# astaka-pe/SeMIGCN

Hardware: AMD Instinct MI355X
Metric: GCN train iters/sec + edges-aggregated/sec, 1M-vert mesh (higher is better)
Workload: dtype bf16 storage / f32 accumulate; 1 GPU; SGCN train iteration (13 ChebConv K=3 + BN + LeakyReLU, fwd+loss+bwd, Adam every 5th) on a closed torus mesh 1000x1000: V=1000000 E=6000000 directed, grid vertex order, bf16 features; V=1000000, E=6000000, vertex_order=grid

## Files before the change

### include/semigcn.h

```cpp
#ifndef SEMIGCN_H
#define SEMIGCN_H

#include <stdint.h>

#ifdef __cplusplus
extern "C" {
#endif

#if defined(__GNUC__)
#define SG_API __attribute__((visibility("default")))
#else
#define SG_API
#endif

#define SG_ABI_VERSION 1

enum sg_status {
  SG_OK = 0,
  SG_ERR_INVALID = -1,
  SG_ERR_HIP = -2,
  SG_ERR_UNSUPPORTED = -3,
  SG_ERR_NO_DEVICE = -4
};

// ... 182 lines not shown
SG_API int64_t sg_bnf_blocks(int64_t F);
SG_API int64_t sg_bnf_scratch_bytes(int64_t F);
SG_API int sg_bnf_filter(const float* pos, const int64_t* faces, const int64_t* f2f, int64_t V, int64_t F, int loop,
                         float sigma_s, const float* start_fn, float* fn, float* n_filtered, float* loss_partial,
                         void* scratch, void* stream);
SG_API int sg_mesh_loss_cad_finalize(const float* partial, int64_t nb, float n_v, float n_f, float w_pos, float k1,
                                     const float* bnf_partial, int64_t nb_bnf, int64_t F, float k2, float* out, void* stream);
SG_API int sg_mesh_loss_cad_bwd_det(const float* pos, const int64_t* faces, const float* target_pos, const float* v_keep,
                                    const float* target_fn, const float* f_keep, const float* fn, const float* n_filtered,
                                    const float* g, int64_t V, int64_t V_ext, int64_t F, const sg_pool* incidence,
                                    float* corner_scratch, float* grad_pos, void* stream);

SG_API int sg_gemm_nt_takes_big_tile(int64_t M, int64_t N, int64_t K, int64_t lda, int64_t ldb, int64_t ldc);
SG_API int64_t sg_gemm_tile_rows(int64_t N);
SG_API int64_t sg_gemm_row_tiles(int64_t M, int64_t N);
SG_API int sg_gemm_nt(const void* A, int64_t lda, const void* B, int64_t ldb, const float* bias, void* C, int64_t ldc,
                      int64_t M, int64_t N, int64_t K, int dtype, float* moments, void* stream);
SG_API int64_t sg_gemm_tn_slabs(int64_t M, int64_t N, int64_t Kp);
SG_API int sg_gemm_tn_takes_big_tile(int64_t M, int64_t N, int64_t Kp, int64_t lda, int64_t ldb);
SG_API int sg_gemm_tn(const void* A, int64_t lda, const void* B, int64_t ldb, int64_t M, int64_t N, int64_t Kp, int dtype,
                      float* workspace, float* out, int64_t ldo, void* stream);
SG_API int sg_gemm_nt_f32_supported(int64_t M, int64_t N, int64_t K, int64_t lda, int64_t ldc);
SG_API int sg_gemm_nt_f32_pays(int64_t M, int64_t N, int64_t K);
SG_API int sg_gemm_nt_f32_variant(int64_t M);
SG_API int64_t sg_gemm_nt_f32_workspace(int64_t N, int64_t K);
SG_API int sg_gemm_nt_f32(const float* A, int64_t lda, const float* W, int64_t w_rs, int64_t w_cs, const float* bias, float* C,
                          int64_t ldc, int64_t M, int64_t N, int64_t K, void* workspace, int64_t workspace_bytes, void* stream);
SG_API int sg_gemm_tn_f32_supported(int64_t M, int64_t N, int64_t Kp, int64_t lda, int64_t ldb);
SG_API int64_t sg_gemm_tn_f32_workspace(int64_t M, int64_t N, int64_t Kp);
SG_API int sg_gemm_tn_f32(const float* A, int64_t lda, const float* B, int64_t ldb, int64_t M, int64_t N, int64_t Kp,
// ... 147 lines not shown
```

### semigcn_amd/capi.py

```python
from __future__ import annotations

import ctypes
import functools
from array import array as _array
import os
from ctypes import POINTER, byref, c_char_p, c_float, c_int, c_int32, c_int64, c_void_p
from typing import Optional

import torch

_LIB_NAME = "libsemigcn_hip.so"
_LIB_PATH = os.path.join(os.path.dirname(os.path.abspath(__file__)), _LIB_NAME)

SG_F32, SG_BF16 = 0, 1
_DTYPES = {torch.float32: SG_F32, torch.bfloat16: SG_BF16}


class SemigcnLibraryError(RuntimeError):
    """libsemigcn_hip.so is absent / unloadable, or a call into it failed."""


class sg_graph_info(ctypes.Structure):
    _fields_ = [("V_dst", c_int64), ("V_src", c_int64), ("nnz", c_int64),
                ("symmetric", c_int32), ("max_degree", c_int32)]
# ... 61 lines not shown
    "sg_tuning_set": (c_int, [c_int, c_int]),
    "sg_mesh_loss_blocks": (c_int64, [c_int64, c_int64]),
    "sg_mesh_loss_fwd": (c_int, [c_void_p] * 6 + [c_int64, c_int64, c_void_p, c_void_p]),
    "sg_mesh_loss_bwd": (c_int, [c_void_p] * 7 + [c_int64, c_int64, c_int64, c_void_p, c_void_p]),
    "sg_mesh_loss_bwd_det": (c_int, [c_void_p] * 7 + [c_int64, c_int64, c_int64, c_void_p, c_void_p, c_void_p, c_void_p]),
    "sg_col_blocks": (c_int64, [c_int64]),
    "sg_col_moments": (c_int, [c_void_p, c_int64, c_int64, c_int64, c_int, c_void_p, c_int64, c_void_p]),
    "sg_bn_merge": (c_int, [c_void_p, c_int64, c_int64, c_int64, c_void_p, c_void_p]),
    "sg_bn_stats_finalize": (c_int, [c_void_p, c_int64, c_int64, c_int64, c_void_p, c_void_p, c_void_p, c_void_p, c_float,
                                     c_float, c_void_p, c_void_p, c_void_p]),
    "sg_bn_stats_finalize_tiles": (c_int, [c_void_p, c_int64, c_int64, c_int64, c_int64, c_void_p, c_void_p, c_void_p,
                                           c_void_p, c_float, c_float, c_void_p, c_void_p, c_void_p]),
    "sg_gemm_nt_takes_big_tile": (c_int, [c_int64, c_int64, c_int64, c_int64, c_int64, c_int64]),
    "sg_gemm_tile_rows": (c_int64, [c_int64]),
    "sg_gemm_row_tiles": (c_int64, [c_int64, c_int64]),
    "sg_gemm_nt": (c_int, [c_void_p, c_int64, c_void_p, c_int64, c_void_p, c_void_p, c_int64, c_int64, c_int64, c_int64,
                           c_int, c_void_p, c_void_p]),
    "sg_gemm_nt_f32_supported": (c_int, [c_int64, c_int64, c_int64, c_int64, c_int64]),
    "sg_gemm_nt_f32_pays": (c_int, [c_int64, c_int64, c_int64]),
    "sg_gemm_nt_f32_variant": (c_int, [c_int64]),
    "sg_gemm_nt_f32_workspace": (c_int64, [c_int64, c_int64]),
    "sg_gemm_nt_f32": (c_int, [c_void_p, c_int64, c_void_p, c_int64, c_int64, c_void_p, c_void_p, c_int64, c_int64, c_int64,
                               c_int64, c_void_p, c_int64, c_void_p]),
    "sg_gemm_tn_f32_supported": (c_int, [c_int64, c_int64, c_int64, c_int64, c_int64]),
    "sg_gemm_tn_f32_workspace": (c_int64, [c_int64, c_int64, c_int64]),
    "sg_gemm_tn_f32": (c_int, [c_void_p, c_int64, c_void_p, c_int64, c_int64, c_int64, c_int64, c_void_p, c_int64, c_void_p,
                               c_int64, c_void_p]),
    "sg_gemm_tn_slabs": (c_int64, [c_int64, c_int64, c_int64]),
    "sg_gemm_tn_takes_big_tile": (c_int, [c_int64, c_int64, c_int64, c_int64, c_int64]),
    "sg_gemm_tn": (c_int, [c_void_p, c_int64, c_void_p, c_int64, c_int64, c_int64, c_int64, c_int, c_void_p, c_void_p, c_int64,
# ... 577 lines not shown
        if t is not None:
            _f32vec(t, C, n)
    with _on_device(partial.device):
        _check(load().sg_bn_stats_finalize_tiles(_ptr(partial), nb, int(rows_per_tile), int(num_rows), C,
                                                 _ptr(_f32vec(gamma, C, "weight")), _ptr(_f32vec(beta, C, "bias")),
                                                 _ptr(running_mean), _ptr(running_var), float(momentum), float(eps),
                                                 _ptr(out), _counter(batches_tracked, partial), _stream(partial)),
               "sg_bn_stats_finalize_tiles")
    return out


def gemm_tile_rows(N: int) -> int:
    return _sizes("sg_gemm_tile_rows", int(N))


def gemm_nt_supported(A: torch.Tensor, B: torch.Tensor, ldc: int) -> bool:
    if A.dtype != torch.bfloat16 or B.dtype != torch.bfloat16 or not A.is_cuda or A.dim() != 2 or B.dim() != 2:
        return False
    if A.shape[1] != B.shape[1] or A.stride(1) != 1 or B.stride(1) != 1 or A.shape[0] == 0:
        return False
    K, N = A.shape[1], B.shape[0]
    return (K % 8 == 0 and N % 8 == 0 and A.stride(0) % 8 == 0 and B.stride(0) % 8 == 0 and ldc % 8 == 0
            and A.data_ptr() % 16 == 0 and B.data_ptr() % 16 == 0)


def gemm_nt_takes_big_tile(M: int, N: int, K: int, lda: int, ldb: int, ldc: int) -> bool:
    return bool(_sizes("sg_gemm_nt_takes_big_tile", int(M), int(N), int(K), int(lda), int(ldb), int(ldc)))


def gemm_nt(A: torch.Tensor, B: torch.Tensor, bias: Optional[torch.Tensor] = None, out: Optional[torch.Tensor] = None,
            moments: bool = False):
    _require_device(A, "A")
    _require_device(B, "B")
    M, K = A.shape
    N = B.shape[0]
    if out is None:
        out = torch.empty((M, N), dtype=torch.bfloat16, device=A.device)
    if out.shape != (M, N) or out.dtype != torch.bfloat16 or B.shape[1] != K:
        raise SemigcnLibraryError(f"gemm_nt shape mismatch: A {tuple(A.shape)} B {tuple(B.shape)} out {tuple(out.shape)}")
    if bias is not None:
        _f32vec(bias, N, "bias")
    mom = None
    if moments:
        mom = torch.empty((_sizes("sg_gemm_row_tiles", M, N), 2, N), dtype=torch.float32, device=A.device)
    with _on_device(A.device):
        _check(load().sg_gemm_nt(_ptr(A), _rows2d(A, "A"), _ptr(B), _rows2d(B, "B"), _ptr(bias), _ptr(out),
                                 _rows2d(out, "out"), M, N, K, SG_BF16, _ptr(mom), _stream(A)), "sg_gemm_nt")
    return (out, mom) if moments else out


THIN_ELEMS = 256


def thin_shape(N: int, K: int) -> bool:
    return bool(_sizes("sg_thin_supported", int(N), int(K)))


def thin_supported(A: torch.Tensor, N: int, K: int) -> bool:
    return (A.is_cuda and A.dim() == 2 and A.stride(1) == 1 and A.dtype in (torch.float32, torch.bfloat16)
# ... 1120 lines not shown
```

### semigcn_amd/csrc/api.hip

```cpp
#include <stdarg.h>

#include <new>

#include <mutex>

#include "sg_common.h"

namespace sg {

static thread_local std::string t_error;

void set_error(const char* fmt, ...) {
  char buf[1024];
  va_list ap;
  va_start(ap, fmt);
  vsnprintf(buf, sizeof(buf), fmt, ap);
  va_end(ap);
  t_error = buf;
}

namespace {

struct ScopedFree {
  void* p = nullptr;
// ... 777 lines not shown
  return launch_bn_stats_finalize_tiles(partial, n_tiles, rows_per_tile, V, C, gamma, beta, running_mean, running_var,
                                        momentum, eps, out, batches_tracked, (hipStream_t)stream);
}

SG_API int sg_gemm_nt_takes_big_tile(int64_t M, int64_t N, int64_t K, int64_t lda, int64_t ldb, int64_t ldc) {
  return gemm_nt_takes_big_tile(M, N, K, lda, ldb, ldc) ? 1 : 0;
}

SG_API int64_t sg_gemm_tile_rows(int64_t N) { return gemm_tile_rows(N); }

SG_API int64_t sg_gemm_row_tiles(int64_t M, int64_t N) {
  const int64_t r = gemm_tile_rows(N);
  return M <= 0 ? 0 : (M + r - 1) / r;
}

SG_API int sg_gemm_nt(const void* A, int64_t lda, const void* B, int64_t ldb, const float* bias, void* C, int64_t ldc,
                      int64_t M, int64_t N, int64_t K, int dtype, float* moments, void* stream) {
  SG_REQUIRE(M >= 0 && N >= 0 && K >= 0, "sg_gemm_nt: negative size");
  if (M == 0 || N == 0) return SG_OK;
  SG_REQUIRE(A && B && C && K > 0, "sg_gemm_nt: null operand or K = 0");
  SG_REQUIRE(lda >= K && ldb >= K && ldc >= N, "sg_gemm_nt: row stride shorter than the row");
  return launch_gemm_nt(A, lda, B, ldb, bias, C, ldc, M, N, K, dtype, moments, (hipStream_t)stream);
}

SG_API int64_t sg_gemm_tn_slabs(int64_t M, int64_t N, int64_t Kp) { return gemm_tn_slabs(M, N, Kp); }

SG_API int sg_gemm_tn_takes_big_tile(int64_t M, int64_t N, int64_t Kp, int64_t lda, int64_t ldb) {
  return gemm_tn_takes_big_tile(M, N, Kp, lda, ldb) ? 1 : 0;
}

// ... 269 lines not shown
```

### semigcn_amd/csrc/block.hip

```cpp
#include <math.h>

#include "sg_common.h"

namespace sg {
namespace {

bool g_block_planes = true;

inline int64_t esize(int dtype) { return dtype == SG_F32 ? 4 : 2; }
inline int64_t align_up(int64_t v) { return (v + 255) & ~(int64_t)255; }

struct Carver {
  char* base;
  int64_t cap, at = 0;
  bool overflow = false;
  Carver(void* b, int64_t c) : base((char*)b), cap(c) {}
  void* take(int64_t bytes) {
    const int64_t off = at;
    at += align_up(bytes > 0 ? bytes : 1);
    if (!base) return nullptr;
    if (at > cap) {
      overflow = true;
      return nullptr;
    }
// ... 47 lines not shown
  if (c >= C) return;
  const float mean = rm[c];
  const float invstd = rsqrtf(__fadd_rn(rv[c], eps));
  const float scale = __fmul_rn(gamma[c], invstd);
  out[c] = mean;
  out[C + c] = invstd;
  out[2 * C + c] = scale;
  out[3 * C + c] = __fsub_rn(beta[c], __fmul_rn(mean, scale));
}

int copy_rows(const void* src, int64_t lds, void* dst, int64_t ldd, int64_t rows, int64_t cols, int dtype, hipStream_t s) {
  const int64_t e = esize(dtype);
  SG_HIP_TRY(hipMemcpy2DAsync(dst, (size_t)(ldd * e), src, (size_t)(lds * e), (size_t)(cols * e), (size_t)rows,
                              hipMemcpyDeviceToDevice, s));
  return SG_OK;
}

struct Shape {
  int64_t V, Vo, Ci, Co, KCi, KCo, e;
  int K;
  bool thin, blas_fwd, blas_dx, blas_dw;
  bool planes_ok;
  Planes pl;
  int64_t nb;
  int64_t mom_floats;
  int64_t tn_floats;
};

int shape_of(const sg_block& b, Shape* s) {
  SG_REQUIRE(b.graph != nullptr, "sg_block: null graph");
// ... 46 lines not shown
    bool ok = b.dtype == SG_BF16 && b.K > 1 && (1 << lg) == C && C >= 8 && C <= 64 && g_block_planes;
    if (ok && b.order == 0)
      ok = dense_planes_ok_nt(b.dtype, s->V, s->Co, s->KCi) && dense_planes_ok_nt(b.dtype, s->V, s->KCi, s->Co) &&
           dense_planes_ok_tn(b.dtype, s->V, s->Co, s->KCi);
    else if (ok)
      ok = dense_planes_ok_nt(b.dtype, s->V, s->KCo, s->Ci) && dense_planes_ok_nt(b.dtype, s->V, s->Ci, s->KCo) &&
           dense_planes_ok_tn(b.dtype, s->V, s->KCo, s->Ci);
    s->planes_ok = ok;
    s->pl = Planes{};
    if (ok) {
      s->pl.log2 = lg;
      s->pl.stride = s->V * C;
    }
  }
  s->nb = col_blocks(s->Vo);
  const int64_t R = gemm_tile_rows(s->Co);
  const int64_t tiles = (s->V + R - 1) / R;
  s->mom_floats = (tiles > s->nb ? tiles : s->nb) * 2 * s->Co;
  return SG_OK;
}

struct FwdWs {
  float* moments;
  void* Z;
  void* Hc;
  void* blas;
};
void carve_fwd(const sg_block& b, const Shape& s, Carver& c, FwdWs* w) {
  w->moments = (float*)c.take(s.mom_floats * 4);
  w->Z = b.order == 1 ? c.take(s.V * s.KCo * s.e) : nullptr;
  w->Hc = b.pool_mode ? c.take(s.V * s.Co * s.e) : nullptr;
  w->blas = s.blas_fwd ? c.take((int64_t)kBlasWorkspace) : nullptr;
// ... 112 lines not shown
    auto z = [&](int k) { return pz.on() ? col(w.Z, k * pz.stride, s.e) : col(w.Z, k * s.Co, s.e); };
    for (int k = b.K - 2; k >= 1; --k) {
      rc = spmm(b, false, z(k + 1), ldz, z(k), ldz, k + 2 <= b.K - 1 ? z(k + 2) : nullptr, ldz, z(k), ldz, s.Co, 2.f, 1.f, -1.f,
                stream);
      if (rc != SG_OK) return rc;
    }
    rc = spmm(b, false, z(1), ldz, z(0), ldz, b.K >= 3 ? z(2) : nullptr, ldz, Hc, s.Co, s.Co, 1.f, 1.f, -1.f, stream);
    if (rc != SG_OK) return rc;
  }
  if (b.pool_mode == 1) rc = sg_pool_mean(b.pool, Hc, s.Co, b.H, s.Co, s.Co, b.dtype, (void*)stream);
  else if (b.pool_mode == 2) rc = sg_unpool(b.pool, Hc, s.Co, b.H, s.Co, s.Co, b.dtype, (void*)stream);
  if (rc != SG_OK) return rc;

  if (b.training) {
    if (tile_moments) {
      const int64_t R = gemm_tile_rows(s.Co);
      rc = launch_bn_stats_finalize_tiles(w.moments, (s.V + R - 1) / R, R, s.Vo, s.Co, b.gamma, b.beta, b.running_mean,
                                          b.running_var, b.momentum, b.eps, b.stats, b.batches_tracked, stream);
    } else {
      rc = launch_col_reduce(0, b.H, s.Co, nullptr, 0, nullptr, nullptr, nullptr, nullptr, 0.f, w.moments, s.nb, s.Vo, s.Co,
                             b.dtype, stream);
      if (rc != SG_OK) return rc;
      rc = launch_bn_stats_finalize(w.moments, s.nb, s.Vo, s.Co, b.gamma, b.beta, b.running_mean, b.running_var, b.momentum,
                                    b.eps, b.stats, b.batches_tracked, stream);
    }
    if (rc != SG_OK) return rc;
  } else {
    bn_eval_coeffs<<<(int)((s.Co + 127) / 128), 128, 0, stream>>>(b.running_mean, b.running_var, b.gamma, b.beta, b.eps,
                                                                 (int)s.Co, b.stats);
    SG_HIP_TRY(hipGetLastError());
  }
// ... 174 lines not shown
  return SG_OK;
}

struct PartWs {
  float* moments;
  void* Z;
  float* part;
  float* co;
  float* colsum;
  void* dH;
  float* tn;
  void* blas;
};
void carve_part(const sg_block& b, Carver& c, PartWs* w) {
  const int64_t e = esize(b.dtype), KCi = b.K * b.Cin, KCo = b.K * b.Cout;
  const int64_t nb = col_blocks(b.V), R = gemm_tile_rows(b.Cout), tiles = (b.V + R - 1) / R;
  w->moments = (float*)c.take((tiles > nb ? tiles : nb) * 2 * b.Cout * 4);
  w->Z = b.order == 1 ? c.take(b.V_ext * KCo * e) : nullptr;
  w->part = (float*)c.take(nb * 2 * b.Cout * 4);
  w->co = (float*)c.take(5 * b.Cout * 4);
  w->colsum = (float*)c.take(col_apply_blocks(b.V, b.Cout, b.dtype) * b.Cout * 4);
  w->dH = b.order == 0 ? c.take(b.V * b.Cout * e) : nullptr;
  const int64_t tn = b.order == 0 ? dense_tn_workspace(b.dtype, b.V, b.Cout, KCi) : dense_tn_workspace(b.dtype, b.V, KCo, b.Cin);
  w->tn = (float*)c.take(tn * 4);
  w->blas = c.take((int64_t)kBlasWorkspace);
}

int pack_to(const sg_block& b, const void* src, int64_t ld, int64_t width, const float* blob, int64_t blob_floats, hipStream_t stream) {
  if (b.n_send == 0) return SG_OK;
  SG_REQUIRE(b.send && b.send_index, "sg_block_run: no send buffer / index");
  const int64_t e = esize(b.dtype);
// ... 37 lines not shown
      if (rc != SG_OK) return rc;
    } else {
      SG_REQUIRE(b.X && b.ldx >= Ci, "sg_block_run (conv): order 1 needs the [V_ext, Cin] input X");
      if (b.bias) SG_REQUIRE(b.bias_k != nullptr, "sg_block_run (conv): order 1 with a bias needs bias_k");
      rc = dense_nt(b.X, b.ldx, b.wpack, nullptr, Ci, b.bias ? b.bias_k : nullptr, w.Z, KCo, Ve, KCo, Ci, b.dtype, nullptr, nullptr,
                    w.blas, kBlasWorkspace, stream, Planes{}, Planes{}, split_image(b, false, KCo, Ci), b.V);
      if (rc != SG_OK) return rc;
      char* z0 = (char*)w.Z;
      char* z1 = col(w.Z, Co, e);
      char* z2 = col(w.Z, 2 * Co, e);
      if ((rc = agg(b.graph_wide, z2, KCo, z1, KCo, nullptr, 0, z1, KCo, Co, 2.f, 1.f, 0.f)) != SG_OK) return rc;
      if ((rc = agg(b.graph, z1, KCo, z0, KCo, z2, KCo, b.H, b.ldh, Co, 1.f, 1.f, -1.f)) != SG_OK) return rc;
    }
    if (b.training) {
      if (tile_moments) {
        const int64_t R = gemm_tile_rows(Co);
        rc = launch_bn_merge_tiles(w.moments, (V + R - 1) / R, R, V, Co, b.local, b.local + 2 * Co, stream);
      } else {
        const int64_t nb = col_blocks(V);
        rc = launch_col_reduce(0, b.H, b.ldh, nullptr, 0, nullptr, nullptr, nullptr, nullptr, 0.f, w.moments, nb, V, Co, b.dtype, stream);
        if (rc != SG_OK) return rc;
        rc = launch_bn_merge_tiles(w.moments, nb, (V + nb - 1) / nb, V, Co, b.local, b.local + 2 * Co, stream);
      }
      if (rc != SG_OK) return rc;
    }
    if (b.n_send > 0 && (rc = pack_to(b, b.H, b.ldh, Co, b.training ? b.local : nullptr, 2 * Co + 1, stream)) != SG_OK) return rc;
  }

  if (b.phase & SG_PHASE_BN) {
    SG_REQUIRE(b.stats && b.gamma && b.beta && b.Y && b.ldy >= Co && b.V_out >= V && b.V_out <= Ve, "sg_block_run (bn): bad argument");
    if (b.training) {
// ... 210 lines not shown
```

### semigcn_amd/csrc/dense.hip

```cpp
#include <dlfcn.h>

#include <map>
#include <mutex>
#include <tuple>

#include <hipblaslt/hipblaslt.h>

#include "sg_common.h"

namespace sg {
namespace {

struct LtApi {
  decltype(&hipblasLtCreate) Create = nullptr;
  decltype(&hipblasLtMatmulDescCreate) DescCreate = nullptr;
  decltype(&hipblasLtMatmulDescSetAttribute) DescSet = nullptr;
  decltype(&hipblasLtMatrixLayoutCreate) LayoutCreate = nullptr;
  decltype(&hipblasLtMatrixLayoutSetAttribute) LayoutSet = nullptr;
  decltype(&hipblasLtMatmulPreferenceCreate) PrefCreate = nullptr;
  decltype(&hipblasLtMatmulPreferenceSetAttribute) PrefSet = nullptr;
  decltype(&hipblasLtMatmulPreferenceDestroy) PrefDestroy = nullptr;
  decltype(&hipblasLtMatmulAlgoGetHeuristic) Heuristic = nullptr;
  decltype(&hipblasLtMatmul) Matmul = nullptr;
  decltype(&hipblasLtGetVersion) GetVersion = nullptr;
// ... 224 lines not shown
  if (moments_done) *moments_done = false;
  if (M == 0 || N == 0) return SG_OK;
  if (pa.on() || pc.on()) {
    SG_REQUIRE(dense_planes_ok_nt(dtype, M, N, K) && a16(A) && a16(Bp) && a16(C),
               "dense_nt: an operand kept as planes for a product the 128-row kernel does not serve (M=%lld N=%lld K=%lld)",
               (long long)M, (long long)N, (long long)K);
    if (moments_done) *moments_done = moments != nullptr;
    TraceScope ts(1, dtype, 1, M, N, K, stream);
    return launch_gemm_nt(A, lda, Bp, ldb, bias, C, ldc, M, N, K, dtype, moments, stream, pa, pc);
  }
  if (thin_shape(N, K) && B32) {
    TraceScope ts(1, dtype, 2, M, N, K, stream);
    return launch_thin_nt(A, lda, B32, ldb, bias, C, ldc, M, N, K, dtype, stream);
  }
  if (dense_nt_own(dtype, M, N, K, lda, ldb, ldc) && a16(A) && a16(Bp) && a16(C)) {
    const bool big = gemm_nt_takes_big_tile(M, N, K, lda, ldb, ldc);
    float* mom = (moments && !big) ? moments : nullptr;
    if (moments_done) *moments_done = mom != nullptr;
    TraceScope ts(1, dtype, 1, M, N, K, stream);
    return launch_gemm_nt(A, lda, Bp, ldb, bias, C, ldc, M, N, K, dtype, mom, stream);
  }
  if (dtype == SG_F32 && split_engine_enabled(0) && split_nt_pays(M, N, K) && gemm_nt_f32s_supported(M, N, K, lda, ldc) && a16(A) && a16(C) &&
      (presplit || (blas_ws && (int64_t)blas_ws_bytes >= gemm_nt_f32s_workspace(N, K)))) {
    TraceScope ts(1, dtype, 4, M, N, K, stream);
    return launch_gemm_nt_f32s((const float*)A, lda, (const float*)Bp, ldb, 1, bias, (float*)C, ldc, M, N, K, blas_ws,
                               (int64_t)blas_ws_bytes, stream, presplit, presplit_rows);
  }
  if (dtype == SG_F32 && split_engine_enabled(0) && mid_shape(N, K) && lda % 4 == 0 && ldc % 4 == 0 && a16(A) && a16(C)) {
    TraceScope ts(1, dtype, 2, M, N, K, stream);
    return launch_mid_nt((const float*)A, lda, (const float*)Bp, ldb, 1, bias, (float*)C, ldc, M, N, K, stream);
  }
  TraceScope ts(1, dtype, 3, M, N, K, stream);
  return lt_gemm(0, 1, M, N, K, A, lda, Bp, ldb, bias, C, ldc, dtype, dtype, 1, 0, 0, 0, blas_ws, blas_ws_bytes, stream);
}

// ... 100 lines not shown
```

### semigcn_amd/csrc/gemm_mfma.hip

```cpp
#include "sg_common.h"

namespace sg {
namespace {

typedef __attribute__((ext_vector_type(8))) __bf16 bf16x8;
typedef __attribute__((ext_vector_type(4))) float f32x4;
typedef uint32_t u32x4 __attribute__((ext_vector_type(4)));

constexpr int kThreads = 256;
constexpr int kBK = 64;
constexpr int kRowBytes = 128;

struct GemmArgs {
  const uint16_t* A; int64_t lda;
  const uint16_t* B; int64_t ldb;
  const float* bias;
  uint16_t* C; int64_t ldc;
  float* moments;
  int M, N, K;
  int n_col_tiles, n_tiles;
  int a_plog; int64_t a_pstride;
  int c_plog; int64_t c_pstride;
};

// ... 233 lines not shown
constexpr int64_t kBigMinWeightElems = 90000;
constexpr int64_t kBigMinRows = 16384;

bool wide_tile(int64_t N) { return g_gemm_tile == 2 && N > 64; }
bool tile_192(int64_t N) { return g_gemm_tile != 1 && g_gemm_tile != 4 && (N == 192 || (g_gemm_tile == 5 && N == 384)); }

}

int gemm_tile_rows(int64_t N) { return wide_tile(N) ? 64 : 128; }

bool gemm_nt_takes_big_tile(int64_t M, int64_t N, int64_t K, int64_t lda, int64_t ldb, int64_t ldc) {
  if (g_gemm_tile == 1 || g_gemm_tile == 2 || !gemm_nt_256_supported(M, N, K, lda, ldb, ldc)) return false;
  return g_gemm_tile == 3 || (K * N > kBigMinWeightElems && M >= kBigMinRows);
}

int set_gemm_tuning(int value) {
  g_gemm_tile = value;
  return SG_OK;
}

int launch_gemm_nt(const void* A, int64_t lda, const void* B, int64_t ldb, const float* bias, void* C, int64_t ldc,
                   int64_t M, int64_t N, int64_t K, int dtype, float* moments, hipStream_t stream, Planes pa, Planes pc) {
  if (dtype != SG_BF16) {
    set_error("sg_gemm_nt: bf16 operands only (dtype %d); fp32 products stay with the BLAS library", dtype);
    return SG_ERR_UNSUPPORTED;
  }
  if (K % 8 || N % 8 || lda % 8 || ldb % 8 || ldc % 8 || !a16(A) || !a16(B) || !a16(C)) {
    set_error("sg_gemm_nt: needs K, N and the row strides to be multiples of 8 and 16-byte aligned operands "
              "(K=%lld N=%lld lda=%lld ldb=%lld ldc=%lld)", (long long)K, (long long)N, (long long)lda, (long long)ldb,
              (long long)ldc);
    return SG_ERR_UNSUPPORTED;
  }
  SG_REQUIRE(M <= INT32_MAX && N <= INT32_MAX && K <= INT32_MAX, "sg_gemm_nt: size out of range");
  const bool planes = pa.on() || pc.on();
  if (planes) {
    SG_REQUIRE((!pa.on() || (pa.log2 >= 3 && pa.log2 < 31 && pa.stride % 8 == 0)) &&
               (!pc.on() || (pc.log2 >= 3 && pc.log2 < 31 && pc.stride % 8 == 0)),
               "sg_gemm_nt: planes need >= 8 columns each and a plane stride that is a multiple of 8 elements");
    SG_REQUIRE(!wide_tile(N), "sg_gemm_nt: operands kept as planes run on the 128-row tiles only");
  }
  if (!planes && moments == nullptr && gemm_nt_takes_big_tile(M, N, K, lda, ldb, ldc))
    return launch_gemm_nt_256(A, lda, B, ldb, bias, C, ldc, M, N, K, stream);
  GemmArgs g;
  g.a_plog = pa.log2; g.a_pstride = pa.stride;
  g.c_plog = pc.log2; g.c_pstride = pc.stride;
  g.A = (const uint16_t*)A; g.lda = lda;
  g.B = (const uint16_t*)B; g.ldb = ldb;
  g.bias = bias;
  g.C = (uint16_t*)C; g.ldc = ldc;
  g.moments = moments;
  g.M = (int)M; g.N = (int)N; g.K = (int)K;
  g.n_col_tiles = g.n_tiles = 0;
  if (wide_tile(N)) return launch<1, 4, 4, 4>(g, stream);
  if (tile_192(N) && !moments) return launch<2, 2, 4, 6>(g, stream);
  if (N > 64) return launch<2, 2, 4, 4>(g, stream);
  if (N > 32) return launch<4, 1, 2, 4>(g, stream);
  if (N > 16) return launch<4, 1, 2, 2>(g, stream);
// ... 247 lines not shown
```

### semigcn_amd/csrc/gemm_mfma256.hip

```cpp
#include "sg_common.h"

namespace sg {
namespace {

typedef __attribute__((ext_vector_type(8))) __bf16 bf16x8;
typedef __attribute__((ext_vector_type(4))) float f32x4;
typedef uint32_t u32x2 __attribute__((ext_vector_type(2)));
typedef uint32_t u32x4 __attribute__((ext_vector_type(4)));
typedef float f32x2 __attribute__((ext_vector_type(2)));
typedef __attribute__((ext_vector_type(4))) __bf16 bf16x4;
typedef __bf16 bf16x2 __attribute__((ext_vector_type(2)));

constexpr int kThreads256 = 512;
constexpr int kHalf = 16384;
constexpr int kBuf = 4 * kHalf;
constexpr int AH0 = 0, AH1 = 1, BH0 = 2, BH1 = 3;

struct Big {
  const uint16_t* A; int64_t lda;
  const uint16_t* B; int64_t ldb;
  const float* bias;
  uint16_t* C; int64_t ldc;
  int M, N, K;
  int n_col_tiles, n_row_tiles, streams;
#ifdef SG_GEMM256_STAMPS
  unsigned long long* stamps;
#endif
};

#if defined(SG_GEMM256_STAMPS) && !defined(SG_G256_NOSTAMP)
#define SG_STAMP(ph, k)                                                                                         \
  if (blockIdx.x == 8 && (wave == 0 || wave == 4) && lane == 0 && s >= 16 && s < 32)                              \
    ((unsigned long long*)(lds + 2 * kBuf))[(((wave >> 2) * 16 + (s - 16)) * 4 + (ph)) * 6 + (k)] = __builtin_readcyclecounter();
#else
#define SG_STAMP(ph, k)
#endif

// ... 33 lines not shown
[[maybe_unused]] __device__ __forceinline__ bf16x8 sg_fake_frag(const uint8_t* p) {
  bf16x8 v;
  asm volatile("" : "=v"(v) : "v"(p));
  return v;
}

__device__ __forceinline__ void glds16(const void* src, uint8_t* lds_dst) {
#ifdef SG_G256_NOLOAD
  asm volatile("" ::"v"(src), "s"(lds_dst));
  return;
#endif
  __builtin_amdgcn_global_load_lds((const void __attribute__((address_space(1)))*)src,
                                   (void __attribute__((address_space(3)))*)lds_dst, 16, 0, 0);
}

__global__ __launch_bounds__(kThreads256, 1) void gemm_nt_256(const Big g) {
#ifdef SG_GEMM256_STAMPS
  __shared__ __attribute__((aligned(1024))) uint8_t lds[2 * kBuf + 2 * 16 * 4 * 6 * 8];
#else
  __shared__ __attribute__((aligned(1024))) uint8_t lds[2 * kBuf];
#endif

  const int tid = threadIdx.x, lane = tid & 63;
  const int wave = __builtin_amdgcn_readfirstlane(tid >> 6);
  const int wr = wave >> 2, wc = wave & 3;
  const int fr = lane & 15, fq = lane >> 4;

  const int b = blockIdx.x;
  const int slot = b >> 3;
  const int ct = slot % g.n_col_tiles;
// ... 84 lines not shown
  load_a(0, 0);
  load_b(0, 0);
  load_b(1, 0);
  load_a(1, 0);
  advance();
  load_a(0, 1);
  load_b(0, 1);
  SG_WAIT_VM(8);
  SG_BARRIER();
  if (wr == 1) SG_BARRIER2();

  int since = 2;
  int pend_row0 = 0;
  auto store_quadrant = [&](int q) {
    const int i0 = q >= 2 ? 4 : 0, jp = (q == 1 || q == 2) ? 1 : 0;
#pragma unroll
    for (int ii = 0; ii < 4; ++ii) {
      const int i = i0 + ii;
      const int row = pend_row0 + (i >> 2) * 128 + wr * 64 + (i & 3) * 16 + fr;
      uint16_t* const cptr = g.C + (int64_t)row * g.ldc + col0 + wc * 32 + (fq & 1) * 16 + (fq >> 1) * 8 + jp * 128;
      uint32_t lo[2], hi[2];
#pragma unroll
      for (int jj = 0; jj < 2; ++jj) {
        const int j = 2 * jp + jj;
        lo[jj] = __builtin_bit_cast(uint32_t, __builtin_convertvector(f32x2{acc[i][j][0], acc[i][j][1]}, bf16x2));
        hi[jj] = __builtin_bit_cast(uint32_t, __builtin_convertvector(f32x2{acc[i][j][2], acc[i][j][3]}, bf16x2));
        acc[i][j] = bias_v[j];
      }
      const auto ra = __builtin_amdgcn_permlane16_swap(lo[0], lo[1], false, false);
      const auto rb = __builtin_amdgcn_permlane16_swap(hi[0], hi[1], false, false);
      if (row < g.M) SG_STORE16(cptr, (u32x4{ra[0], rb[0], ra[1], rb[1]}));
    }
  };
#define SG_PHASE_WAIT(n0, n1)                 \
  if (since == 0) SG_WAIT_VM(n0);             \
  else SG_WAIT_VM(n1);

  bf16x8 af[4][2], bf0[2][2], bf1[2][2];
  int ct_k = 0, ct_t = 0;
  for (int s = 0; s < total; ++s) {
    const int buf = s & 1;
    const uint8_t* const base = lds + buf * kBuf;
    SG_STAMP(0, 0)
#pragma unroll
    for (int j = 0; j < 2; ++j)
#pragma unroll
      for (int ks = 0; ks < 2; ++ks) bf0[j][ks] = SG_LDS_FRAG(base + BH0 * kHalf + b_rd[ks] + j * 2048);
#pragma unroll
    for (int i = 0; i < 4; ++i)
#pragma unroll
      for (int ks = 0; ks < 2; ++ks) af[i][ks] = SG_LDS_FRAG(base + AH0 * kHalf + a_rd[ks] + i * 2048);
// ... 286 lines not shown
#pragma unroll
      for (int r = 0; r < 4; ++r) {
        const int n = n0 + (i >> 2) * 128 + wr * 64 + (i & 3) * 16 + fg * 4 + r;
        W[(int64_t)n * g.Kp + kk] = acc[i][j][r];
      }
    }
}

}

bool gemm_nt_256_supported(int64_t M, int64_t N, int64_t K, int64_t lda, int64_t ldb, int64_t ldc) {
  return K >= 128 && K % 64 == 0 && N >= 256 && N % 256 == 0 && M >= 256 && lda % 8 == 0 && ldb % 8 == 0 && ldc % 8 == 0 &&
         256 * lda * 2 < (int64_t)1 << 31 && 256 * ldb * 2 < (int64_t)1 << 31;
}

int launch_gemm_nt_256(const void* A, int64_t lda, const void* B, int64_t ldb, const float* bias, void* C, int64_t ldc,
                       int64_t M, int64_t N, int64_t K, hipStream_t stream) {
  SG_REQUIRE(gemm_nt_256_supported(M, N, K, lda, ldb, ldc), "sg_gemm_nt (256-tile kernel): unsupported shape");
  SG_REQUIRE((((uintptr_t)A | (uintptr_t)B) & 15) == 0 && ((uintptr_t)C & 15) == 0, "sg_gemm_nt (256-tile kernel): misaligned operand");
  Big g;
  g.A = (const uint16_t*)A; g.lda = lda;
  g.B = (const uint16_t*)B; g.ldb = ldb;
  g.bias = bias;
  g.C = (uint16_t*)C; g.ldc = ldc;
  g.M = (int)M; g.N = (int)N; g.K = (int)K;
  g.n_col_tiles = (int)(N / 256);
  g.n_row_tiles = (int)((M + 255) / 256);
  int dev = 0, cus = 256;
  SG_HIP_TRY(hipGetDevice(&dev));
  SG_HIP_TRY(hipDeviceGetAttribute(&cus, hipDeviceAttributeMultiprocessorCount, dev));
  int streams = (cus / g.n_col_tiles) / 8 * 8;
  streams = streams < 8 ? 8 : streams;
  const int need = (g.n_row_tiles + 7) / 8 * 8;
  streams = streams > need ? need : streams;
  g.streams = streams;
  gemm_nt_256<<<streams * g.n_col_tiles, kThreads256, 0, stream>>>(g);
  SG_HIP_TRY(hipGetLastError());
  return SG_OK;
}

bool gemm_tn_256_supported(int64_t M, int64_t N, int64_t Kp, int64_t lda, int64_t ldb) {
  return M >= 64 * 64 && N >= 256 && N % 256 == 0 && Kp >= 256 && Kp % 256 == 0 && lda % 8 == 0 && ldb % 8 == 0 &&
         64 * lda * 2 < (int64_t)1 << 31 && 64 * ldb * 2 < (int64_t)1 << 31;
}

int gemm_tn_256_slabs(int64_t M, int64_t N, int64_t Kp) {
  const int n_tiles = (int)((N / 256) * (Kp / 256));
  int slabs = (256 / n_tiles) / 8 * 8;
  slabs = slabs < 8 ? 8 : slabs;
  const int64_t steps = M / 64;
  while (slabs > 8 && steps < slabs) slabs -= 8;
// ... 22 lines not shown
```

### semigcn_amd/csrc/sg_common.h

```cpp
#pragma once
#include <hip/hip_runtime.h>
#include <stdint.h>
#include <stdio.h>
#include <atomic>
#include <string>

#include "semigcn.h"

namespace sg {

void set_error(const char* fmt, ...);

#define SG_HIP_TRY(expr)                                                              \
  do {                                                                                \
    hipError_t e__ = (expr);                                                          \
    if (e__ != hipSuccess) {                                                          \
      sg::set_error("%s failed: %s (%s:%d)", #expr, hipGetErrorString(e__), __FILE__, \
                    __LINE__);                                                        \
      return SG_ERR_HIP;                                                              \
    }                                                                                 \
  } while (0)

#define SG_REQUIRE(cond, ...)      \
  do {                             \
// ... 194 lines not shown
int launch_input_prep_bwd(const void* gX, int64_t ldg, const float* z1, const float* dm, const int64_t* rank, const float* lo,
                          const float* hi, float* dz1, float* partial, float* d_lo, float* d_hi, int64_t V, int dtype,
                          hipStream_t stream);

int launch_input_bounds(const float* z1, int64_t V, float* pv, int64_t* pi, float* bounds, int64_t* arg, hipStream_t stream);
int launch_bounds_route(const float* d_lo, const float* d_hi, const int64_t* arg, float* dz1, hipStream_t stream);
int launch_mesh_loss_finalize(const float* partial, int64_t nb, float n_v, float n_f, float w_pos, float k1, float* out,
                              hipStream_t stream);

int gemm_tile_rows(int64_t N);
int set_gemm_tuning(int value);
int launch_gemm_nt(const void* A, int64_t lda, const void* B, int64_t ldb, const float* bias, void* C, int64_t ldc,
                   int64_t M, int64_t N, int64_t K, int dtype, float* moments, hipStream_t stream, Planes pa = {}, Planes pc = {});

bool gemm_nt_takes_big_tile(int64_t M, int64_t N, int64_t K, int64_t lda, int64_t ldb, int64_t ldc);
bool gemm_nt_256_supported(int64_t M, int64_t N, int64_t K, int64_t lda, int64_t ldb, int64_t ldc);
int launch_gemm_nt_256(const void* A, int64_t lda, const void* B, int64_t ldb, const float* bias, void* C, int64_t ldc,
                       int64_t M, int64_t N, int64_t K, hipStream_t stream);
bool gemm_tn_256_supported(int64_t M, int64_t N, int64_t Kp, int64_t lda, int64_t ldb);
int gemm_tn_256_slabs(int64_t M, int64_t N, int64_t Kp);
int launch_gemm_tn_256(const void* A, int64_t lda, const void* B, int64_t ldb, int64_t M, int64_t N, int64_t Kp,
                       float* workspace, hipStream_t stream);
bool gemm_tn_takes_big_tile(int64_t M, int64_t N, int64_t Kp, int64_t lda, int64_t ldb);
int64_t gemm_tn_slabs(int64_t M, int64_t N, int64_t Kp);
int launch_gemm_tn(const void* A, int64_t lda, const void* B, int64_t ldb, int64_t M, int64_t N, int64_t Kp, int dtype,
                   float* workspace, float* out, int64_t ldo, hipStream_t stream, const GradSink* sink = nullptr, Planes pa = {},
                   Planes pb = {});

bool gemm_nt_f32s_supported(int64_t M, int64_t N, int64_t K, int64_t lda, int64_t ldc);
int64_t gemm_nt_f32s_workspace(int64_t N, int64_t K);
int launch_gemm_nt_f32s(const float* A, int64_t lda, const float* W, int64_t w_rs, int64_t w_cs, const float* bias, float* C,
                        int64_t ldc, int64_t M, int64_t N, int64_t K, void* ws, int64_t ws_bytes, hipStream_t stream,
                        const void* prepacked = nullptr, int64_t variant_rows = 0);
// ... 145 lines not shown
```

### semigcn_amd/functional.py

```python
from __future__ import annotations

import contextlib
import os
import weakref
from typing import Optional, Sequence

import torch

from . import capi
from .graph import MeshGraph


def _mm_f32_out(a: torch.Tensor, b: torch.Tensor) -> torch.Tensor:
    if a.dtype == torch.float32:
        return a @ b
    try:
        return torch.mm(a, b, out_dtype=torch.float32)
    except (TypeError, RuntimeError):
        return (a @ b).float()


def _bmm_f32_out(a: torch.Tensor, b: torch.Tensor) -> torch.Tensor:
    if a.dtype == torch.float32:
        return torch.bmm(a, b)
# ... 278 lines not shown
    if _gemm_timer is None or not a.is_cuda:
        return _dense_nt(a, b, bias, out, moments)
    ldc = b.shape[0] if out is None else out.stride(0)
    own = _mfma_ok(a, b, ldc) and (out is None or (out.stride(1) == 1 and out.data_ptr() % 16 == 0))
    engine = "mfma" if own else ("thin" if _thin_ok(a, b.shape[0], a.shape[1], out) else
                                 ("split" if _nt_split(a, b.shape[0], out) and b.dtype == torch.float32 else "blas"))
    with _timed(("nt", a.shape[0], b.shape[0], a.shape[1], str(a.dtype).replace("torch.", ""), engine)):
        return _dense_nt(a, b, bias, out, moments)


def _dense_nt(a: torch.Tensor, b: torch.Tensor, bias: Optional[torch.Tensor] = None, out: Optional[torch.Tensor] = None,
              moments: Optional[dict] = None) -> torch.Tensor:
    ldc = b.shape[0] if out is None else out.stride(0)
    if _mfma_ok(a, b, ldc) and (out is None or (out.stride(1) == 1 and out.data_ptr() % 16 == 0)):
        bias32 = None if bias is None else (bias if bias.dtype == torch.float32 else bias.float()).contiguous()
        if moments is not None and not _mfma_big(a, b, ldc):
            res, mom = capi.gemm_nt(a, b, bias32, out=out, moments=True)
            moments["tiles"], moments["rows"] = mom, capi.gemm_tile_rows(b.shape[0])
            return res
        return capi.gemm_nt(a, b, bias32, out=out)
    if _thin_ok(a, b.shape[0], a.shape[1], out):
        bias32 = None if bias is None else (bias if bias.dtype == torch.float32 else bias.float()).contiguous()
        return capi.thin_nt(a, b, bias32, out=out)
    if b.dtype == torch.float32 and b.dim() == 2 and _nt_split(a, b.shape[0], out):
        return capi.gemm_nt_f32(a, b, None if bias is None else bias.float().contiguous(), out=out)
    if bias is not None:
        return torch.addmm(bias.to(a.dtype), a, b.t()) if out is None else torch.addmm(bias.to(a.dtype), a, b.t(), out=out)
    return a @ b.t() if out is None else torch.mm(a, b.t(), out=out)


def dense_nn(a: torch.Tensor, w: torch.Tensor, out: Optional[torch.Tensor] = None) -> torch.Tensor:
    thin = a.is_cuda and a.dim() == 2 and w.dim() == 2 and _thin_ok(a, w.shape[1], a.shape[1], out)
    split = (not thin) and w.dim() == 2 and w.dtype == torch.float32 and _nt_split(a, w.shape[1], out)
# ... 1059 lines not shown
```

Baseline: 38.35 iter/s.

## Fuse BatchNorm moment accumulation into the 256-tile MFMA GEMM epilogue

The big-tile 256-row GEMM kernel now optionally computes per-64-row shifted column moments (sum and sum of squares around a median pivot) in its store epilogue, using DPP cross-lane reductions. Previously, requesting moments forced the slower 128-row tile or a separate column-moments pass over the output. Moment record sizing and finalize/merge calls now use a kernel-dependent row granularity. The cost is extra epilogue ALU work, more registers and a changed VM wait count in the moments variant, which may lower the throughput of the big-tile kernel.

```diff
diff --git a/include/semigcn.h b/include/semigcn.h
--- a/include/semigcn.h
+++ b/include/semigcn.h
@@ -220,6 +220,7 @@
 SG_API int sg_gemm_nt_takes_big_tile(int64_t M, int64_t N, int64_t K, int64_t lda, int64_t ldb, int64_t ldc);
 SG_API int64_t sg_gemm_tile_rows(int64_t N);
 SG_API int64_t sg_gemm_row_tiles(int64_t M, int64_t N);
+SG_API int64_t sg_gemm_nt_moment_rows(int64_t M, int64_t N, int64_t K, int64_t lda, int64_t ldb, int64_t ldc);
 SG_API int sg_gemm_nt(const void* A, int64_t lda, const void* B, int64_t ldb, const float* bias, void* C, int64_t ldc,
                       int64_t M, int64_t N, int64_t K, int dtype, float* moments, void* stream);
 SG_API int64_t sg_gemm_tn_slabs(int64_t M, int64_t N, int64_t Kp);
diff --git a/semigcn_amd/capi.py b/semigcn_amd/capi.py
--- a/semigcn_amd/capi.py
+++ b/semigcn_amd/capi.py
@@ -99,6 +99,7 @@
     "sg_gemm_nt_takes_big_tile": (c_int, [c_int64, c_int64, c_int64, c_int64, c_int64, c_int64]),
     "sg_gemm_tile_rows": (c_int64, [c_int64]),
     "sg_gemm_row_tiles": (c_int64, [c_int64, c_int64]),
+    "sg_gemm_nt_moment_rows": (c_int64, [c_int64, c_int64, c_int64, c_int64, c_int64, c_int64]),
     "sg_gemm_nt": (c_int, [c_void_p, c_int64, c_void_p, c_int64, c_void_p, c_void_p, c_int64, c_int64, c_int64, c_int64,
                            c_int, c_void_p, c_void_p]),
     "sg_gemm_nt_f32_supported": (c_int, [c_int64, c_int64, c_int64, c_int64, c_int64]),
@@ -706,6 +707,10 @@
     return _sizes("sg_gemm_tile_rows", int(N))
 
 
+def gemm_nt_moment_rows(M: int, N: int, K: int, lda: int, ldb: int, ldc: int) -> int:
+    return _sizes("sg_gemm_nt_moment_rows", int(M), int(N), int(K), int(lda), int(ldb), int(ldc))
+
+
 def gemm_nt_supported(A: torch.Tensor, B: torch.Tensor, ldc: int) -> bool:
     if A.dtype != torch.bfloat16 or B.dtype != torch.bfloat16 or not A.is_cuda or A.dim() != 2 or B.dim() != 2:
         return False
@@ -734,7 +739,8 @@
         _f32vec(bias, N, "bias")
     mom = None
     if moments:
-        mom = torch.empty((_sizes("sg_gemm_row_tiles", M, N), 2, N), dtype=torch.float32, device=A.device)
+        R = gemm_nt_moment_rows(M, N, K, _rows2d(A, "A"), _rows2d(B, "B"), _rows2d(out, "out"))
+        mom = torch.empty(((M + R - 1) // R, 2, N), dtype=torch.float32, device=A.device)
     with _on_device(A.device):
         _check(load().sg_gemm_nt(_ptr(A), _rows2d(A, "A"), _ptr(B), _rows2d(B, "B"), _ptr(bias), _ptr(out),
                                  _rows2d(out, "out"), M, N, K, SG_BF16, _ptr(mom), _stream(A)), "sg_gemm_nt")
diff --git a/semigcn_amd/csrc/api.hip b/semigcn_amd/csrc/api.hip
--- a/semigcn_amd/csrc/api.hip
+++ b/semigcn_amd/csrc/api.hip
@@ -815,6 +815,10 @@
   return M <= 0 ? 0 : (M + r - 1) / r;
 }
 
+SG_API int64_t sg_gemm_nt_moment_rows(int64_t M, int64_t N, int64_t K, int64_t lda, int64_t ldb, int64_t ldc) {
+  return gemm_nt_moment_rows(M, N, K, lda, ldb, ldc);
+}
+
 SG_API int sg_gemm_nt(const void* A, int64_t lda, const void* B, int64_t ldb, const float* bias, void* C, int64_t ldc,
                       int64_t M, int64_t N, int64_t K, int dtype, float* moments, void* stream) {
   SG_REQUIRE(M >= 0 && N >= 0 && K >= 0, "sg_gemm_nt: negative size");
diff --git a/semigcn_amd/csrc/block.hip b/semigcn_amd/csrc/block.hip
--- a/semigcn_amd/csrc/block.hip
+++ b/semigcn_amd/csrc/block.hip
@@ -85,6 +85,15 @@
   SG_HIP_TRY(hipMemcpy2DAsync(dst, (size_t)(ldd * e), src, (size_t)(lds * e), (size_t)(cols * e), (size_t)rows,
                               hipMemcpyDeviceToDevice, s));
   return SG_OK;
+}
+
+inline int64_t conv_moment_rows(const sg_block& b, int64_t ldh) {
+  return gemm_nt_moment_rows(b.V, b.Cout, b.K * b.Cin, b.ldt, b.K * b.Cin, ldh);
+}
+inline int64_t conv_moment_records(const sg_block& b, int64_t ldh) {
+  const int64_t a = gemm_nt_moment_rows(b.V, b.Cout, b.K * b.Cin, b.K * b.Cin, b.K * b.Cin, ldh), c = gemm_tile_rows(b.Cout);
+  const int64_t R = a < c ? a : c;
+  return (b.V + R - 1) / R;
 }
 
 struct Shape {
@@ -161,8 +170,7 @@
     }
   }
   s->nb = col_blocks(s->Vo);
-  const int64_t R = gemm_tile_rows(s->Co);
-  const int64_t tiles = (s->V + R - 1) / R;
+  const int64_t tiles = conv_moment_records(b, s->Co);
   s->mom_floats = (tiles > s->nb ? tiles : s->nb) * 2 * s->Co;
   return SG_OK;
 }
@@ -305,7 +313,7 @@
 
   if (b.training) {
     if (tile_moments) {
-      const int64_t R = gemm_tile_rows(s.Co);
+      const int64_t R = conv_moment_rows(b, s.Co);
       rc = launch_bn_stats_finalize_tiles(w.moments, (s.V + R - 1) / R, R, s.Vo, s.Co, b.gamma, b.beta, b.running_mean,
                                           b.running_var, b.momentum, b.eps, b.stats, b.batches_tracked, stream);
     } else {
@@ -510,7 +518,7 @@
 };
 void carve_part(const sg_block& b, Carver& c, PartWs* w) {
   const int64_t e = esize(b.dtype), KCi = b.K * b.Cin, KCo = b.K * b.Cout;
-  const int64_t nb = col_blocks(b.V), R = gemm_tile_rows(b.Cout), tiles = (b.V + R - 1) / R;
+  const int64_t nb = col_blocks(b.V), tiles = conv_moment_records(b, b.Cout);
   w->moments = (float*)c.take((tiles > nb ? tiles : nb) * 2 * b.Cout * 4);
   w->Z = b.order == 1 ? c.take(b.V_ext * KCo * e) : nullptr;
   w->part = (float*)c.take(nb * 2 * b.Cout * 4);
@@ -578,7 +586,7 @@
     }
     if (b.training) {
       if (tile_moments) {
-        const int64_t R = gemm_tile_rows(Co);
+        const int64_t R = conv_moment_rows(b, b.ldh);
         rc = launch_bn_merge_tiles(w.moments, (V + R - 1) / R, R, V, Co, b.local, b.local + 2 * Co, stream);
       } else {
         const int64_t nb = col_blocks(V);
diff --git a/semigcn_amd/csrc/dense.hip b/semigcn_amd/csrc/dense.hip
--- a/semigcn_amd/csrc/dense.hip
+++ b/semigcn_amd/csrc/dense.hip
@@ -262,11 +262,9 @@
     return launch_thin_nt(A, lda, B32, ldb, bias, C, ldc, M, N, K, dtype, stream);
   }
   if (dense_nt_own(dtype, M, N, K, lda, ldb, ldc) && a16(A) && a16(Bp) && a16(C)) {
-    const bool big = gemm_nt_takes_big_tile(M, N, K, lda, ldb, ldc);
-    float* mom = (moments && !big) ? moments : nullptr;
-    if (moments_done) *moments_done = mom != nullptr;
+    if (moments_done) *moments_done = moments != nullptr;
     TraceScope ts(1, dtype, 1, M, N, K, stream);
-    return launch_gemm_nt(A, lda, Bp, ldb, bias, C, ldc, M, N, K, dtype, mom, stream);
+    return launch_gemm_nt(A, lda, Bp, ldb, bias, C, ldc, M, N, K, dtype, moments, stream);
   }
   if (dtype == SG_F32 && split_engine_enabled(0) && split_nt_pays(M, N, K) && gemm_nt_f32s_supported(M, N, K, lda, ldc) && a16(A) && a16(C) &&
       (presplit || (blas_ws && (int64_t)blas_ws_bytes >= gemm_nt_f32s_workspace(N, K)))) {
diff --git a/semigcn_amd/csrc/gemm_mfma.hip b/semigcn_amd/csrc/gemm_mfma.hip
--- a/semigcn_amd/csrc/gemm_mfma.hip
+++ b/semigcn_amd/csrc/gemm_mfma.hip
@@ -271,6 +271,10 @@
   return g_gemm_tile == 3 || (K * N > kBigMinWeightElems && M >= kBigMinRows);
 }
 
+int gemm_nt_moment_rows(int64_t M, int64_t N, int64_t K, int64_t lda, int64_t ldb, int64_t ldc) {
+  return gemm_nt_takes_big_tile(M, N, K, lda, ldb, ldc) ? gemm_nt_256_moment_rows() : gemm_tile_rows(N);
+}
+
 int set_gemm_tuning(int value) {
   g_gemm_tile = value;
   return SG_OK;
@@ -296,8 +300,8 @@
                "sg_gemm_nt: planes need >= 8 columns each and a plane stride that is a multiple of 8 elements");
     SG_REQUIRE(!wide_tile(N), "sg_gemm_nt: operands kept as planes run on the 128-row tiles only");
   }
-  if (!planes && moments == nullptr && gemm_nt_takes_big_tile(M, N, K, lda, ldb, ldc))
-    return launch_gemm_nt_256(A, lda, B, ldb, bias, C, ldc, M, N, K, stream);
+  if (!planes && gemm_nt_takes_big_tile(M, N, K, lda, ldb, ldc))
+    return launch_gemm_nt_256(A, lda, B, ldb, bias, C, ldc, M, N, K, moments, stream);
   GemmArgs g;
   g.a_plog = pa.log2; g.a_pstride = pa.stride;
   g.c_plog = pc.log2; g.c_pstride = pc.stride;
diff --git a/semigcn_amd/csrc/gemm_mfma256.hip b/semigcn_amd/csrc/gemm_mfma256.hip
--- a/semigcn_amd/csrc/gemm_mfma256.hip
+++ b/semigcn_amd/csrc/gemm_mfma256.hip
@@ -21,6 +21,7 @@
   const uint16_t* B; int64_t ldb;
   const float* bias;
   uint16_t* C; int64_t ldc;
+  float* moments;
   int M, N, K;
   int n_col_tiles, n_row_tiles, streams;
 #ifdef SG_GEMM256_STAMPS
@@ -84,6 +85,24 @@
                                    (void __attribute__((address_space(3)))*)lds_dst, 16, 0, 0);
 }
 
+constexpr int kMomentRows = 64;
+constexpr int kDppRowLane0 = 0x150;
+constexpr int kDppMirror = 0x140, kDppHalfMirror = 0x141;
+constexpr int kDppXor2 = 0x4E, kDppXor1 = 0xB1;
+
+template <int CTRL>
+__device__ __forceinline__ float dpp_get(float v) {
+  return __builtin_bit_cast(float, __builtin_amdgcn_update_dpp(0, __builtin_bit_cast(int, v), CTRL, 0xf, 0xf, true));
+}
+__device__ __forceinline__ float row_first(float v) {
+  return dpp_get<kDppRowLane0>(v);
+}
+template <int CTRL>
+__device__ __forceinline__ float dpp_halve(float a, float b, bool up) {
+  return (up ? b : a) + dpp_get<CTRL>(up ? a : b);
+}
+
+template <bool MOMENTS>
 __global__ __launch_bounds__(kThreads256, 1) void gemm_nt_256(const Big g) {
 #ifdef SG_GEMM256_STAMPS
   __shared__ __attribute__((aligned(1024))) uint8_t lds[2 * kBuf + 2 * 16 * 4 * 6 * 8];
@@ -198,6 +217,21 @@
   int pend_row0 = 0;
   auto store_quadrant = [&](int q) {
     const int i0 = q >= 2 ? 4 : 0, jp = (q == 1 || q == 2) ? 1 : 0;
+    [[maybe_unused]] f32x2 s1[2][2], s2[2][2], kk[2][2];
+    if constexpr (MOMENTS) {
+#pragma unroll
+      for (int jj = 0; jj < 2; ++jj)
+#pragma unroll
+        for (int h = 0; h < 2; ++h) {
+          const int j = 2 * jp + jj;
+          const float m0 = __builtin_amdgcn_fmed3f(acc[i0][j][2 * h], acc[i0 + 1][j][2 * h], acc[i0 + 2][j][2 * h]);
+          const float m1 = __builtin_amdgcn_fmed3f(acc[i0][j][2 * h + 1], acc[i0 + 1][j][2 * h + 1], acc[i0 + 2][j][2 * h + 1]);
+          const uint32_t w = __builtin_bit_cast(uint32_t, __builtin_convertvector(f32x2{m0, m1}, bf16x2));
+          kk[jj][h] = f32x2{row_first(__uint_as_float(w << 16)), row_first(__uint_as_float(w & 0xffff0000u))};
+          s1[jj][h] = f32x2{0.f, 0.f};
+          s2[jj][h] = f32x2{0.f, 0.f};
+        }
+    }
 #pragma unroll
     for (int ii = 0; ii < 4; ++ii) {
       const int i = i0 + ii;
@@ -211,14 +245,59 @@
         hi[jj] = __builtin_bit_cast(uint32_t, __builtin_convertvector(f32x2{acc[i][j][2], acc[i][j][3]}, bf16x2));
         acc[i][j] = bias_v[j];
       }
+      if constexpr (MOMENTS) {
+        const float on = row < g.M ? 1.f : 0.f;
+        const f32x2 on2 = {on, on};
+#pragma unroll
+        for (int jj = 0; jj < 2; ++jj)
+#pragma unroll
+          for (int h = 0; h < 2; ++h) {
+            const uint32_t w = h ? hi[jj] : lo[jj];
+            const f32x2 v = {__uint_as_float(w << 16), __uint_as_float(w & 0xffff0000u)};
+            const f32x2 d = (v - kk[jj][h]) * on2;
+            s1[jj][h] += d;
+            s2[jj][h] = __builtin_elementwise_fma(d, d, s2[jj][h]);
+          }
+      }
       const auto ra = __builtin_amdgcn_permlane16_swap(lo[0], lo[1], false, false);
       const auto rb = __builtin_amdgcn_permlane16_swap(hi[0], hi[1], false, false);
       if (row < g.M) SG_STORE16(cptr, (u32x4{ra[0], rb[0], ra[1], rb[1]}));
     }
+    if constexpr (MOMENTS) {
+      const bool b3 = fr & 8, b2 = fr & 4, b1 = fr & 2, odd = fr & 1;
+      float t1[4], t2[4], tk[4];
+#pragma unroll
+      for (int e = 0; e < 4; ++e) {
+        t1[e] = dpp_halve<kDppMirror>(s1[0][e >> 1][e & 1], s1[1][e >> 1][e & 1], b3);
+        t2[e] = dpp_halve<kDppMirror>(s2[0][e >> 1][e & 1], s2[1][e >> 1][e & 1], b3);
+        tk[e] = b3 ? kk[1][e >> 1][e & 1] : kk[0][e >> 1][e & 1];
+      }
+      float u1[2], u2[2], uk[2];
+#pragma unroll
+      for (int e = 0; e < 2; ++e) {
+        u1[e] = dpp_halve<kDppHalfMirror>(t1[e], t1[2 + e], b2);
+        u2[e] = dpp_halve<kDppHalfMirror>(t2[e], t2[2 + e], b2);
+        uk[e] = b2 ? tk[2 + e] : tk[e];
+      }
+      float w1 = dpp_halve<kDppXor2>(u1[0], u1[1], b1), w2 = dpp_halve<kDppXor2>(u2[0], u2[1], b1);
+      const float wk = b1 ? uk[1] : uk[0];
+      w1 += dpp_get<kDppXor1>(w1);
+      w2 += dpp_get<kDppXor1>(w2);
+      const int rec_row0 = pend_row0 + (q >= 2 ? 128 : 0) + wr * kMomentRows;
+      const int n = g.M - rec_row0 < kMomentRows ? g.M - rec_row0 : kMomentRows;
+      if (n > 0) {
+        const float nf = (float)n;
+        const float r = (odd ? fmaf(nf, w2, -(w1 * w1)) : w1) / nf;
+        const int col = col0 + jp * 128 + wc * 32 + (fr >> 3) * 16 + fq * 4 + ((fr >> 1) & 3);
+        g.moments[((int64_t)(rec_row0 / kMomentRows) * 2 + (odd ? 1 : 0)) * g.N + col] = odd ? fmaxf(r, 0.f) : wk + r;
+      }
+    }
   };
 #define SG_PHASE_WAIT(n0, n1)                 \
-  if (since == 0) SG_WAIT_VM(n0);             \
-  else SG_WAIT_VM(n1);
+  if (since == 0) {                           \
+    if constexpr (MOMENTS) SG_WAIT_VM(28);    \
+    else SG_WAIT_VM(n0);                      \
+  } else SG_WAIT_VM(n1);
 
   bf16x8 af[4][2], bf0[2][2], bf1[2][2];
   int ct_k = 0, ct_t = 0;
@@ -535,8 +614,10 @@
          256 * lda * 2 < (int64_t)1 << 31 && 256 * ldb * 2 < (int64_t)1 << 31;
 }
 
+int gemm_nt_256_moment_rows() { return kMomentRows; }
+
 int launch_gemm_nt_256(const void* A, int64_t lda, const void* B, int64_t ldb, const float* bias, void* C, int64_t ldc,
-                       int64_t M, int64_t N, int64_t K, hipStream_t stream) {
+                       int64_t M, int64_t N, int64_t K, float* moments, hipStream_t stream) {
   SG_REQUIRE(gemm_nt_256_supported(M, N, K, lda, ldb, ldc), "sg_gemm_nt (256-tile kernel): unsupported shape");
   SG_REQUIRE((((uintptr_t)A | (uintptr_t)B) & 15) == 0 && ((uintptr_t)C & 15) == 0, "sg_gemm_nt (256-tile kernel): misaligned operand");
   Big g;
@@ -544,6 +625,7 @@
   g.B = (const uint16_t*)B; g.ldb = ldb;
   g.bias = bias;
   g.C = (uint16_t*)C; g.ldc = ldc;
+  g.moments = moments;
   g.M = (int)M; g.N = (int)N; g.K = (int)K;
   g.n_col_tiles = (int)(N / 256);
   g.n_row_tiles = (int)((M + 255) / 256);
@@ -555,7 +637,8 @@
   const int need = (g.n_row_tiles + 7) / 8 * 8;
   streams = streams > need ? need : streams;
   g.streams = streams;
-  gemm_nt_256<<<streams * g.n_col_tiles, kThreads256, 0, stream>>>(g);
+  if (moments) gemm_nt_256<true><<<streams * g.n_col_tiles, kThreads256, 0, stream>>>(g);
+  else gemm_nt_256<false><<<streams * g.n_col_tiles, kThreads256, 0, stream>>>(g);
   SG_HIP_TRY(hipGetLastError());
   return SG_OK;
 }
diff --git a/semigcn_amd/csrc/sg_common.h b/semigcn_amd/csrc/sg_common.h
--- a/semigcn_amd/csrc/sg_common.h
+++ b/semigcn_amd/csrc/sg_common.h
@@ -232,9 +232,11 @@
                    int64_t M, int64_t N, int64_t K, int dtype, float* moments, hipStream_t stream, Planes pa = {}, Planes pc = {});
 
 bool gemm_nt_takes_big_tile(int64_t M, int64_t N, int64_t K, int64_t lda, int64_t ldb, int64_t ldc);
+int gemm_nt_moment_rows(int64_t M, int64_t N, int64_t K, int64_t lda, int64_t ldb, int64_t ldc);
 bool gemm_nt_256_supported(int64_t M, int64_t N, int64_t K, int64_t lda, int64_t ldb, int64_t ldc);
+int gemm_nt_256_moment_rows();
 int launch_gemm_nt_256(const void* A, int64_t lda, const void* B, int64_t ldb, const float* bias, void* C, int64_t ldc,
-                       int64_t M, int64_t N, int64_t K, hipStream_t stream);
+                       int64_t M, int64_t N, int64_t K, float* moments, hipStream_t stream);
 bool gemm_tn_256_supported(int64_t M, int64_t N, int64_t Kp, int64_t lda, int64_t ldb);
 int gemm_tn_256_slabs(int64_t M, int64_t N, int64_t Kp);
 int launch_gemm_tn_256(const void* A, int64_t lda, const void* B, int64_t ldb, int64_t M, int64_t N, int64_t Kp,
diff --git a/semigcn_amd/functional.py b/semigcn_amd/functional.py
--- a/semigcn_amd/functional.py
+++ b/semigcn_amd/functional.py
@@ -316,9 +316,10 @@
     ldc = b.shape[0] if out is None else out.stride(0)
     if _mfma_ok(a, b, ldc) and (out is None or (out.stride(1) == 1 and out.data_ptr() % 16 == 0)):
         bias32 = None if bias is None else (bias if bias.dtype == torch.float32 else bias.float()).contiguous()
-        if moments is not None and not _mfma_big(a, b, ldc):
+        if moments is not None:
             res, mom = capi.gemm_nt(a, b, bias32, out=out, moments=True)
-            moments["tiles"], moments["rows"] = mom, capi.gemm_tile_rows(b.shape[0])
+            moments["tiles"] = mom
+            moments["rows"] = capi.gemm_nt_moment_rows(a.shape[0], b.shape[0], a.shape[1], a.stride(0), b.stride(0), ldc)
             return res
         return capi.gemm_nt(a, b, bias32, out=out)
     if _thin_ok(a, b.shape[0], a.shape[1], out):
```

Result: no change. 38.54 iter/s, median of 6 (+0.5%).
